# jolars/sgdnet

Hardware: AMD Instinct MI355X
Metric: saga_epochs_per_sec (higher is better)
Workload: dtype f64

## Files before the change

### include/sgdnet_hip.h

```cpp
#ifndef SGDNET_HIP_H_
#define SGDNET_HIP_H_

#include <stdint.h>

#ifdef __cplusplus
extern "C" {
#endif

#define SGDNET_ABI_VERSION 6

#define SGDNET_OK          0
#define SGDNET_EINVAL     -1
#define SGDNET_ENODEVICE  -2
#define SGDNET_EHIP       -3
#define SGDNET_ENOMEM     -4
#define SGDNET_EUNSUPPORTED -5
#define SGDNET_ESTREAM    -6

#define SGDNET_GAUSSIAN    0
#define SGDNET_BINOMIAL    1
#define SGDNET_MULTINOMIAL 2
#define SGDNET_MGAUSSIAN   3

#define SGDNET_RIDGE       0
// ... 119 lines not shown
int sgdnet_solver_set_penalty(sgdnet_solver* s, int penalty, double gamma, double alpha, double beta);

int sgdnet_solver_get_state(sgdnet_solver* s, int which, double* host);
int sgdnet_solver_set_state(sgdnet_solver* s, int which, const double* host);

int sgdnet_solver_generate_stream(sgdnet_solver* s, sgdnet_rng* rng, int64_t count);

int sgdnet_solver_get_stream(sgdnet_solver* s, uint32_t* host, int64_t offset, int64_t count);

int sgdnet_solver_upload_stream(sgdnet_solver* s, const uint32_t* host, int64_t count);

int sgdnet_solver_run(sgdnet_solver* s, int mode, int64_t batch,
                      int64_t stream_offset, int64_t draws_per_epoch,
                      unsigned max_epochs, double tol,
                      unsigned* epochs_run, int* converged, double* losses);

int sgdnet_solver_enqueue_epochs(sgdnet_solver* s, int64_t batch, int64_t stream_offset,
                                 int64_t draws_per_epoch, int n_epochs);
int sgdnet_solver_sync(sgdnet_solver* s);

int sgdnet_solver_rng_layout(sgdnet_solver* s, int64_t draws_per_run);
int sgdnet_solver_rng_open(sgdnet_solver* s, sgdnet_rng* rng, int64_t draws_per_epoch, int generators);
int sgdnet_solver_rng_next(sgdnet_solver* s, int64_t* stream_offset);
int sgdnet_solver_rng_done(sgdnet_solver* s);
int sgdnet_solver_rng_close(sgdnet_solver* s, sgdnet_rng* rng);

int sgdnet_solver_profile_epoch(sgdnet_solver* s, int64_t batch, int64_t stream_offset,
                                int64_t draws_per_epoch, double* gather_ms, int* gather_launches,
                                double* sweep_ms, int* sweep_launches);

int sgdnet_solver_epoch_timing(sgdnet_solver* s, int enable, double* sum_ms, int* launches);

int sgdnet_solver_gather_form(const sgdnet_solver* s, int64_t batch);

int sgdnet_solver_link_peers(sgdnet_solver** solvers, int n);
int sgdnet_solver_peer_info_bytes(void);
int sgdnet_solver_peer_info(sgdnet_solver* s, void* out);
int sgdnet_solver_link_ipc(sgdnet_solver* s, int rank, int n_ranks, const void* infos);
int sgdnet_solver_set_cu_budget(sgdnet_solver* s, int cus);

int sgdnet_solver_deviance(sgdnet_solver* s, double* out);

int sgdnet_solver_snapshot(sgdnet_solver* s);
int sgdnet_solver_export_delta(sgdnet_solver* s, void* device_buf);
int sgdnet_solver_apply_merged(sgdnet_solver* s, const void* device_buf, double w_weight);
int64_t sgdnet_solver_delta_len(const sgdnet_solver* s);

void* sgdnet_solver_stream(sgdnet_solver* s);
int sgdnet_solver_export_delta_async(sgdnet_solver* s, void* device_buf);
int sgdnet_solver_export_delta_weighted_async(sgdnet_solver* s, void* device_buf, double weight);
int sgdnet_solver_apply_merged_async(sgdnet_solver* s, const void* device_buf, double w_weight);

int64_t sgdnet_solver_sync_buffer_len(const sgdnet_solver* s);
int sgdnet_solver_sync_bind(sgdnet_solver* s, void* device_buf);
int sgdnet_solver_sync_begin(sgdnet_solver* s, int64_t stream_offset, int64_t draws_local_per_epoch);
int sgdnet_solver_sync_gather(sgdnet_solver* s, int64_t t0_local, int64_t m_local, int round);
int sgdnet_solver_sync_sweep(sgdnet_solver* s, int64_t m_global, int64_t m_local, int round);
int sgdnet_solver_sync_end(sgdnet_solver* s, int rounds);

int sgdnet_solver_set_virtual_shards(sgdnet_solver* s, int n_shards);
int sgdnet_solver_set_merge_period(sgdnet_solver* s, int64_t draws_per_shard);

int sgdnet_solver_set_n_total(sgdnet_solver* s, int64_t n_total);

int sgdnet_solver_convergence(sgdnet_solver* s, double tol, int* converged);

// ... 132 lines not shown
```

### sgdnet_amd/_lib.py

```python
import ctypes as C
import os
import sys

_HERE = os.path.dirname(os.path.abspath(__file__))
LIB_PATH = os.environ.get("SGDNET_LIB_PATH") or os.path.join(_HERE, "lib", "libsgdnet_hip.so")

EXPORTS = [
    "sgdnet_abi_version", "sgdnet_last_error", "sgdnet_device_count", "sgdnet_set_option", "sgdnet_get_option",
    "sgdnet_fit_sparse", "sgdnet_fit_dense",
    "sgdnet_rng_seed", "sgdnet_rng_unif", "sgdnet_rng_fill", "sgdnet_rng_jump_poly", "sgdnet_rng_jump",
    "sgdnet_solver_create", "sgdnet_solver_destroy", "sgdnet_solver_set_penalty",
    "sgdnet_solver_get_state", "sgdnet_solver_set_state", "sgdnet_solver_upload_stream",
    "sgdnet_solver_generate_stream", "sgdnet_solver_get_stream",
    "sgdnet_solver_run", "sgdnet_solver_enqueue_epochs", "sgdnet_solver_sync",
    "sgdnet_solver_profile_epoch", "sgdnet_solver_deviance", "sgdnet_solver_snapshot",
    "sgdnet_solver_export_delta", "sgdnet_solver_apply_merged", "sgdnet_solver_delta_len",
    "sgdnet_solver_convergence", "sgdnet_solver_last_change", "sgdnet_auto_batch", "sgdnet_shard_window",
    "sgdnet_solver_gather_form", "sgdnet_solver_stream", "sgdnet_solver_export_delta_async",
    "sgdnet_solver_apply_merged_async", "sgdnet_solver_sync_buffer_len", "sgdnet_solver_sync_bind",
    "sgdnet_solver_sync_begin", "sgdnet_solver_sync_gather", "sgdnet_solver_sync_sweep",
    "sgdnet_solver_sync_end", "sgdnet_solver_set_n_total",
    "sgdnet_solver_export_delta_weighted_async", "sgdnet_solver_set_virtual_shards", "sgdnet_solver_set_merge_period",
    "sgdnet_score_sparse", "sgdnet_score_dense", "sgdnet_predict_sparse", "sgdnet_predict_dense",
    "sgdnet_auc_sparse", "sgdnet_auc_dense", "sgdnet_auc_sparse_rng", "sgdnet_auc_dense_rng",
    "sgdnet_solver_link_peers", "sgdnet_solver_set_cu_budget", "sgdnet_solver_epoch_timing",
    "sgdnet_solver_peer_info_bytes", "sgdnet_solver_peer_info", "sgdnet_solver_link_ipc",
    "sgdnet_solver_rng_layout", "sgdnet_solver_rng_open", "sgdnet_solver_rng_next", "sgdnet_solver_rng_done", "sgdnet_solver_rng_close",
    "sgdnet_gradient_sparse", "sgdnet_gradient_dense", "sgdnet_covariance_max_features",
    "sgdnet_setup_probe_sparse", "sgdnet_setup_probe_dense",
    "sgdnet_cv_covariance_dense", "sgdnet_cv_covariance_sparse", "sgdnet_newton_max_features",
    "sgdnet_newton_probe_dense", "sgdnet_newton_probe_sparse",
    "sgdnet_cv_newton_dense", "sgdnet_cv_newton_sparse", "sgdnet_mcovariance_max_features",
    "sgdnet_mnewton_max_features",
]
ABI_VERSION = 6
MEASURES = {"deviance": 0, "mse": 1, "mae": 2, "class": 3, "auc": 4}

FAMILIES = {"gaussian": 0, "binomial": 1, "multinomial": 2, "mgaussian": 3}
PENALTIES = {"ridge": 0, "elasticnet": 1, "grouplasso": 2}
MODES = {"exact": 0, "batched": 1, "auto": 2, "covariance": 3}
MODE_NEWTON = 4
MODE_MCOVARIANCE = 5
MODE_MNEWTON = 6

UNIF_FN = C.CFUNCTYPE(C.c_double, C.c_void_p)
LOSSES_FN = C.CFUNCTYPE(None, C.c_void_p, C.c_int, C.POINTER(C.c_double), C.c_int)


class Csc(C.Structure):
    _fields_ = [("n_rows", C.c_int64), ("n_cols", C.c_int64),
                ("colptr", C.POINTER(C.c_int32)), ("rowidx", C.POINTER(C.c_int32)),
                ("values", C.POINTER(C.c_double))]


class Rng(C.Structure):
    _fields_ = [("mti", C.c_uint32), ("mt", C.c_uint32 * 624)]


class Control(C.Structure):
    _fields_ = [("debug", C.c_int), ("elasticnet_mix", C.c_double), ("family", C.c_int),
                ("intercept", C.c_int), ("is_sparse", C.c_int),
                ("lambda_", C.POINTER(C.c_double)), ("n_lambda_user", C.c_int),
                ("lambda_min_ratio", C.c_double), ("max_iter", C.c_uint), ("n_lambda", C.c_int),
                ("n_classes", C.c_int), ("standardize", C.c_int),
                ("standardize_response", C.c_int), ("tol", C.c_double),
                ("type_multinomial", C.c_int),
# ... 103 lines not shown
    L.sgdnet_solver_enqueue_epochs.argtypes = [C.c_void_p, C.c_int64, C.c_int64, C.c_int64, C.c_int]
    L.sgdnet_solver_sync.argtypes = [C.c_void_p]
    L.sgdnet_solver_profile_epoch.argtypes = [C.c_void_p, C.c_int64, C.c_int64, C.c_int64,
                                              C.POINTER(C.c_double), C.POINTER(C.c_int),
                                              C.POINTER(C.c_double), C.POINTER(C.c_int)]
    L.sgdnet_solver_deviance.argtypes = [C.c_void_p, C.POINTER(C.c_double)]
    L.sgdnet_solver_snapshot.argtypes = [C.c_void_p]
    L.sgdnet_solver_export_delta.argtypes = [C.c_void_p, C.c_void_p]
    L.sgdnet_solver_apply_merged.argtypes = [C.c_void_p, C.c_void_p, C.c_double]
    L.sgdnet_solver_delta_len.argtypes = [C.c_void_p]
    L.sgdnet_solver_stream.argtypes = [C.c_void_p]
    L.sgdnet_solver_stream.restype = C.c_void_p
    L.sgdnet_solver_export_delta_async.argtypes = [C.c_void_p, C.c_void_p]
    L.sgdnet_solver_apply_merged_async.argtypes = [C.c_void_p, C.c_void_p, C.c_double]
    L.sgdnet_solver_sync_buffer_len.argtypes = [C.c_void_p]
    L.sgdnet_solver_sync_buffer_len.restype = C.c_int64
    L.sgdnet_solver_sync_bind.argtypes = [C.c_void_p, C.c_void_p]
    L.sgdnet_solver_sync_begin.argtypes = [C.c_void_p, C.c_int64, C.c_int64]
    L.sgdnet_solver_sync_gather.argtypes = [C.c_void_p, C.c_int64, C.c_int64, C.c_int]
    L.sgdnet_solver_sync_sweep.argtypes = [C.c_void_p, C.c_int64, C.c_int64, C.c_int]
    L.sgdnet_solver_sync_end.argtypes = [C.c_void_p, C.c_int]
    L.sgdnet_solver_set_n_total.argtypes = [C.c_void_p, C.c_int64]
    L.sgdnet_solver_set_virtual_shards.argtypes = [C.c_void_p, C.c_int]
    L.sgdnet_solver_set_merge_period.argtypes = [C.c_void_p, C.c_int64]
    L.sgdnet_solver_link_peers.argtypes = [C.POINTER(C.c_void_p), C.c_int]
    L.sgdnet_solver_set_cu_budget.argtypes = [C.c_void_p, C.c_int]
    L.sgdnet_solver_peer_info.argtypes = [C.c_void_p, C.c_void_p]
    L.sgdnet_solver_link_ipc.argtypes = [C.c_void_p, C.c_int, C.c_int, C.c_void_p]
    L.sgdnet_solver_epoch_timing.argtypes = [C.c_void_p, C.c_int, C.POINTER(C.c_double), C.POINTER(C.c_int)]
    L.sgdnet_solver_export_delta_weighted_async.argtypes = [C.c_void_p, C.c_void_p, C.c_double]
    L.sgdnet_solver_convergence.argtypes = [C.c_void_p, C.c_double, C.POINTER(C.c_int)]
    L.sgdnet_solver_last_change.argtypes = [C.c_void_p, C.POINTER(C.c_double), C.POINTER(C.c_double)]
    L.sgdnet_solver_gather_form.argtypes = [C.c_void_p, C.c_int64]
    L.sgdnet_auto_batch.argtypes = [C.c_double, C.c_double]
    L.sgdnet_auto_batch.restype = C.c_int64
    L.sgdnet_shard_window.argtypes = [C.c_int64, C.c_int64]
    L.sgdnet_shard_window.restype = C.c_int64
    L.sgdnet_fit_sparse.argtypes = [C.POINTER(Csc), C.POINTER(C.c_double), C.c_int,
                                    C.POINTER(Control), C.POINTER(Result)]
    L.sgdnet_fit_dense.argtypes = [C.POINTER(C.c_double), C.c_int64, C.c_int64,
                                   C.POINTER(C.c_double), C.c_int, C.POINTER(Control),
                                   C.POINTER(Result)]
    L.sgdnet_rng_fill.argtypes = [C.POINTER(Rng), C.c_uint32, C.POINTER(C.c_uint32), C.c_int64]
    L.sgdnet_solver_rng_open.argtypes = [C.c_void_p, C.POINTER(Rng), C.c_int64, C.c_int]
    L.sgdnet_solver_rng_layout.argtypes = [C.c_void_p, C.c_int64]
    L.sgdnet_solver_rng_next.argtypes = [C.c_void_p, C.POINTER(C.c_int64)]
    L.sgdnet_solver_rng_done.argtypes = [C.c_void_p]
    L.sgdnet_solver_rng_close.argtypes = [C.c_void_p, C.POINTER(Rng)]
    L.sgdnet_rng_jump_poly.argtypes = [C.c_uint64, C.POINTER(C.c_uint32)]
    L.sgdnet_rng_jump.argtypes = [C.POINTER(Rng), C.POINTER(C.c_uint32), C.POINTER(Rng)]
    L.sgdnet_rng_jump.restype = None
    _grad_tail = [C.POINTER(C.c_double), C.c_int, C.c_int, C.c_int, C.POINTER(C.c_double), C.POINTER(C.c_double),
                  C.c_int, C.c_int, C.POINTER(C.c_double), C.POINTER(C.c_double)]
    L.sgdnet_gradient_sparse.argtypes = [C.POINTER(Csc)] + _grad_tail
    L.sgdnet_gradient_dense.argtypes = [C.POINTER(C.c_double), C.c_int64, C.c_int64] + _grad_tail
    L.sgdnet_setup_probe_sparse.argtypes = [C.POINTER(Csc), C.c_int, C.POINTER(C.c_double), C.c_int, C.POINTER(C.c_double),
                                            C.c_int, C.c_int, C.c_int, C.POINTER(SetupProbe)]
    L.sgdnet_setup_probe_dense.argtypes = [C.POINTER(C.c_double), C.c_int64, C.c_int64, C.c_int, C.POINTER(C.c_double), C.c_int,
                                           C.c_int64, C.c_int64, C.c_int, C.POINTER(SetupProbe)]
    L.sgdnet_newton_probe_dense.argtypes = [C.POINTER(C.c_double), C.c_int64, C.c_int64, C.c_int, C.POINTER(NewtonProbe)]
    L.sgdnet_newton_probe_sparse.argtypes = [C.POINTER(Csc), C.c_int, C.POINTER(NewtonProbe)]
    _cv_tail = [C.POINTER(C.c_double), C.POINTER(C.c_int32), C.c_int, C.c_int, C.POINTER(Control), C.c_int, C.POINTER(C.c_double),
                C.POINTER(C.c_double), C.POINTER(CvCovResult)]
    L.sgdnet_cv_covariance_dense.argtypes = [C.POINTER(C.c_double), C.c_int64, C.c_int64] + _cv_tail
    L.sgdnet_cv_covariance_sparse.argtypes = [C.POINTER(Csc)] + _cv_tail
    _cv_tail = _cv_tail[:-1] + [C.POINTER(CvNewtonResult)]
# ... 16 lines not shown
```

### sgdnet_amd/csrc/batched_geometry.hpp

```cpp
#pragma once

#include <hip/hip_ext.h>

#include <type_traits>

#include "common.hpp"

#ifndef SGDNET_BIN_BLOCK
#define SGDNET_BIN_BLOCK 1024
#endif
#ifndef SGDNET_BIN_W
#define SGDNET_BIN_W 8
#endif
#ifndef SGDNET_RANGE_BLOCK
#define SGDNET_RANGE_BLOCK 512
#endif
#ifndef SGDNET_LDS_BLOCK
#define SGDNET_LDS_BLOCK 1024
#endif

namespace sgdnet {

constexpr int kGroup = 16;
constexpr int kBlock = 256;

constexpr int kD0Slots = 256;

constexpr int kCStride = 128;
constexpr uint32_t kIdMask = 0x1fffffffu;
constexpr int kInReg8 = 16;

constexpr int kLdsBlock = SGDNET_LDS_BLOCK;
constexpr int kDenseBlock = 256;
constexpr int kDenseVsBlock = 1024;
constexpr int kTileF = 64;

constexpr int kSlabElems = 32;
constexpr int kSlabGroups = kBlock / kSlabElems;

constexpr int kSyncLine = 32;
constexpr int kSyncGo = 0, kSyncExit = 1, kSyncStart = 2, kSyncCnt1 = 3, kSyncCnt2 = kSyncCnt1 + 8,
              kSyncXcd = kSyncCnt2 + 8;
constexpr int kFusedMaxBps = 128;
constexpr int kSyncLines = kSyncXcd + 8;
constexpr int kSyncSticky = kSyncLines;
constexpr int kSyncSeq = kSyncLines + 1;
constexpr int kFusedChunks = 3;
constexpr long long kFusedStartTicks = 2000000;
constexpr long long kFusedWaitTicks = 200000000;

struct __attribute__((aligned(16))) BinEntry {
  uint32_t t;
  uint32_t j;
  double x;
};
static_assert(sizeof(BinEntry) == 16, "bin entries are 16 bytes");

constexpr int kBinBlock = SGDNET_BIN_BLOCK;
constexpr int kBinDraws = kBinBlock / 2;
constexpr int kBinEntCap = 7 * kBinBlock;
constexpr int kBinW = SGDNET_BIN_W;
constexpr int kRangeBlock = SGDNET_RANGE_BLOCK;
constexpr size_t kRangeLdsBytes = 64 * 1024;

constexpr size_t kLdsPerCu = 160 * 1024;
constexpr size_t kLdsStaticReserve = 2 * 1024;
constexpr size_t kLdsTableMax = 80 * 1024;
constexpr int kLdsCap = 96 * 1024;
constexpr int kLdsAll = (int)(kLdsPerCu - kLdsStaticReserve);

template <typename F>
static int with_class_width(int kw, F&& f) {
  if (kw == 1) return f(std::integral_constant<int, 1>{});
  if (kw == 4) return f(std::integral_constant<int, 4>{});
  return f(std::integral_constant<int, 16>{});
}

static inline unsigned clamped_grid(int64_t work, int64_t per_block, int64_t most) {
  const int64_t grid = (work + per_block - 1) / per_block;
// ... 32 lines not shown
```

### sgdnet_amd/csrc/batched_plan.cpp

```cpp
#include <mutex>
#include <set>
#include <utility>

#include "batched_geometry.hpp"
#include "r_rng_bodies.hpp"

namespace sgdnet {

int batched_max_classes() { return 64; }

int lds_target_grid(const SagaDev& d) {
  static const int forced = exp_env_int("SGDNET_LDS_GRID", 0);
  if (forced > 0) return forced;
  const int cus = d.cu_budget > 0 && d.cu_budget < 256 ? d.cu_budget : 256;
  const int g = cus - d.cu_reserve;
  return g < 64 ? 64 : g;
}

size_t binned_max_range_features(int K) { return kRangeLdsBytes / (sizeof(double) * (size_t)K); }

static size_t table_bytes(const SagaDev& d) { return sizeof(double) * (size_t)d.K * (size_t)d.p; }

int allow_dynamic_lds(const void* kernel, int bytes) {
  int dev = 0;
// ... 16 lines not shown

bool compact_eligible(const SagaDev& d) {
  static const int allow = exp_env_int("SGDNET_COMPACT", 1);
  if (!allow || d.K != 1 || d.Ky != 1 || d.xd || !d.ptr || d.p > 65536) return false;
  if (2 * sizeof(double) * (size_t)d.p + 16 + kLdsStaticReserve > (size_t)kLdsPerCu) return false;
  return (double)d.n * 2.0 * kCStride <= 48e9 && d.n < (int64_t)kIdMask;
}

int compact_entries(const SagaDev& d) { return d.family == SGDNET_BINOMIAL && d.y_binary ? 12 : 11; }

bool wants_binned(const SagaDev& d, int64_t batch) {
  static const int allow = exp_env_int("SGDNET_BINNED", 1);
  return allow && !d.xd && d.rec && d.idx && d.K <= 64 && !d.force_global && d.p < (1ll << 31) &&
         (d.K > 16 || (table_bytes(d) > kLdsTableMax && batch >= 4096));
}

bool wants_tiles(const SagaDev& d) { return d.xd && d.K <= 64 && (d.K > 16 || table_bytes(d) > kLdsTableMax); }

bool vs_eligible(const SagaDev& d) {
  if (d.V < 2 || d.K < 1 || d.K > 16 || (d.standardize && !(d.vcw && d.c)) || d.force_global || !d.vw) return false;
  const size_t table = table_bytes(d);
  if (d.xd) return table <= kLdsTableMax;
  if (d.K > 1) return d.rec && table <= kLdsTableMax;
  return 2 * table + 16 + kLdsStaticReserve <= kLdsPerCu;
}

static int vs_grid(const SagaDev& d) { return d.v_bps * d.V; }

static int64_t fused_slice(const SagaDev& d) { return 2 * ((d.p + 2 * (int64_t)d.v_bps - 1) / (2 * (int64_t)d.v_bps)); }
static size_t fused_lds_bytes(const SagaDev& d) {
  const int64_t part = (int64_t)(kLdsBlock / 64) * fused_slice(d);
  return sizeof(double) * (size_t)(d.p + (part > d.p ? part : d.p)) + 16;
}
size_t vs_fused_sync_words() { return (size_t)(kSyncLines + 2) * kSyncLine; }
size_t vs_fused_sync_sticky_word() { return (size_t)kSyncSticky * kSyncLine; }
size_t vs_fused_col_words() { return (size_t)kFusedMaxBps * kSyncLine; }
size_t vs_fused_exchange_doubles(const SagaDev& d, int n_shards) {
  return (size_t)n_shards * (size_t)(2 * d.p + 2) + (size_t)n_shards * kFusedMaxBps;
}
size_t vs_fused_publish_doubles(const SagaDev& d, int n_shards) { return (size_t)2 * n_shards * (size_t)(2 * d.p + 2); }

bool vs_fused_eligible(const SagaDev& d) {
  if (!vs_eligible(d) || d.K != 1 || d.xd || !d.cP || !lanes8_ok(d) || (d.p & 1) || !d.vsync || !d.vx || !d.vcol || !d.vpub) return false;
  if (d.v_bps < 1 || d.v_bps > kFusedMaxBps || d.V * d.v_bps > 1024) return false;
  if (fused_slice(d) > 2 * 64 * kFusedChunks) return false;
  if ((int64_t)d.V * d.v_bps * d.p * 8 >= (1ll << 31)) return false;
  return fused_lds_bytes(d) + kLdsStaticReserve <= kLdsPerCu;
}

static int vs_fused_rng_workgroups(const SagaDev& d) { return d.rngdev ? d.cu_reserve : 0; }

BatchPlan plan_batch(const SagaDev& d, int m, const PlanInputs& in) {
  BatchPlan g{};
  g.kw = class_width(d.K);
  const size_t table = table_bytes(d);
  if (d.V > 1 && vs_eligible(d)) {
    const int rng_wgs = vs_fused_rng_workgroups(d);
    g.slab_doubles = (int64_t)vs_grid(d) * d.K * d.p;
    if (in.fused && vs_fused_eligible(d) && vs_grid(d) + rng_wgs <= in.cus) {
      g.form = BatchForm::kFusedEpoch;
      g.grid = vs_grid(d) + rng_wgs;
      g.lds_bytes = fused_lds_bytes(d);
      if (rng_wgs > 0 && g.lds_bytes < kJumpLds) g.lds_bytes = kJumpLds;
      return g;
    }
    g.form = BatchForm::kShards;
    g.grid = vs_grid(d);
    int dpb = (m + d.v_bps - 1) / d.v_bps;
// ... 88 lines not shown
```

### sgdnet_amd/csrc/batched_shards.hip

```cpp
#include "batched_k1.hpp"
#include "r_rng_bodies.hpp"

namespace sgdnet {

template <int KMAX>
__global__ __launch_bounds__(kBlock) void saga_vs_sweep_kernel(SagaDev d, LamParams* lamp, int tail, int nfb) {
  __shared__ double part[kSlabGroups][kSlabElems];
  __shared__ double red[kBlock / 64];
  __shared__ double sh_d0[KMAX];
  const SweepParams q = load_sweep_params(d, lamp, tail, SweepOverride{0.0, 0.0, 0.0});
  const int K = KMAX == 1 ? 1 : d.K;
  const int F = kSlabElems / K;
  const int E = F * K;
  const int v = (int)blockIdx.x / nfb, fb = (int)blockIdx.x - v * nfb;
  const int64_t KP = (int64_t)K * d.p;
  const double n_d = d.v_size[v];
  const int e = threadIdx.x % kSlabElems, g = threadIdx.x / kSlabElems;
  const int64_t elem = (int64_t)fb * E + e;
  const int64_t j_own = (int64_t)fb * F + threadIdx.x;
  const bool updates = (int)threadIdx.x < F && j_own < d.p;
  double w_old[KMAX], g_old[KMAX], c_own = 0.0;
#pragma unroll
  for (int k = 0; k < KMAX; ++k) {
    w_old[k] = g_old[k] = 0.0;
// ... 172 lines not shown
}
__device__ __forceinline__ unsigned sync_load(unsigned* sync, int word) {
  return __hip_atomic_load(sync + word * kSyncLine, __ATOMIC_RELAXED, __HIP_MEMORY_SCOPE_AGENT);
}

__device__ __forceinline__ void fused_arrive(unsigned* sync, int word) {
  asm volatile("s_waitcnt vmcnt(0)" ::: "memory");
  __syncthreads();
  if (threadIdx.x == 0)
    __hip_atomic_fetch_add(sync + word * kSyncLine, 1u, __ATOMIC_RELAXED, __HIP_MEMORY_SCOPE_AGENT);
}

__device__ __forceinline__ bool fused_poll(unsigned* ctr, int word, unsigned target, LamParams* lamp, bool system = false,
                                           unsigned* sync = nullptr) {
  if (!sync) sync = ctr;
  const long long t0 = wall_clock64();
  for (unsigned spins = 1;; ++spins) {
    const unsigned now = system ? __hip_atomic_load(ctr + word * kSyncLine, __ATOMIC_RELAXED, __HIP_MEMORY_SCOPE_SYSTEM)
                                : sync_load(ctr, word);
    if (now >= target) return true;
    __builtin_amdgcn_s_sleep(4);
    if ((spins & 63u) == 0) {
      if (sync_load(sync, kSyncGo) != 1u) return false;
      if (wall_clock64() - t0 > kFusedWaitTicks) {
        __hip_atomic_store(sync + kSyncGo * kSyncLine, 3u, __ATOMIC_RELAXED, __HIP_MEMORY_SCOPE_AGENT);
        __hip_atomic_store(&lamp->fused_abort, 2, __ATOMIC_RELAXED, __HIP_MEMORY_SCOPE_AGENT);
        __hip_atomic_store(sync + kSyncSticky * kSyncLine, 2u, __ATOMIC_RELAXED, __HIP_MEMORY_SCOPE_AGENT);
        return false;
      }
    }
  }
}

__device__ __forceinline__ bool fused_start(unsigned* sync, LamParams* lamp, unsigned grid) {
  unsigned* go = sync + kSyncGo * kSyncLine;
  const long long t0 = wall_clock64();
  if (blockIdx.x == 0) {
    unsigned expect = 0u;
    for (;;) {
      if (sync_load(sync, kSyncStart) >= grid) {
        __hip_atomic_compare_exchange_strong(go, &expect, 1u, __ATOMIC_RELAXED, __ATOMIC_RELAXED, __HIP_MEMORY_SCOPE_AGENT);
        break;
      }
      if (sync_load(sync, kSyncGo) != 0u) break;
      if (wall_clock64() - t0 > kFusedStartTicks) {
        __hip_atomic_compare_exchange_strong(go, &expect, 2u, __ATOMIC_RELAXED, __ATOMIC_RELAXED, __HIP_MEMORY_SCOPE_AGENT);
        break;
      }
      __builtin_amdgcn_s_sleep(4);
    }
  } else {
    for (;;) {
      if (sync_load(sync, kSyncGo) != 0u) break;
      if (wall_clock64() - t0 > 2 * kFusedStartTicks) {
        unsigned expect = 0u;
        __hip_atomic_compare_exchange_strong(go, &expect, 2u, __ATOMIC_RELAXED, __ATOMIC_RELAXED, __HIP_MEMORY_SCOPE_AGENT);
        break;
      }
      __builtin_amdgcn_s_sleep(4);
    }
  }
  const unsigned decision = sync_load(sync, kSyncGo);
  if (decision != 1u && decision != 3u) {
    __hip_atomic_store(&lamp->fused_abort, 1, __ATOMIC_RELAXED, __HIP_MEMORY_SCOPE_AGENT);
    __hip_atomic_fetch_max(sync + kSyncSticky * kSyncLine, 1u, __ATOMIC_RELAXED, __HIP_MEMORY_SCOPE_AGENT);
  }
  return decision == 1u;
}

__device__ __forceinline__ double fused_block_sum(double a, double* red) {
  a = wave_sum(a);
  if ((threadIdx.x & 63) == 0) red[threadIdx.x >> 6] = a;
  __syncthreads();
  double t = 0.0;
#pragma unroll
  for (int wv = 0; wv < kLdsBlock / 64; ++wv) t += red[wv];
  __syncthreads();
  return t;
}

__device__ __forceinline__ void fused_leave(const SagaDev& d, LamParams* lamp, int nb, bool epoch_done) {
  asm volatile("s_waitcnt vmcnt(0)" ::: "memory");
  __syncthreads();
  if (threadIdx.x == 0) {
    unsigned* sync = d.vsync;
    if (epoch_done && blockIdx.x == 0) {
      end_epoch(lamp, nb);
      if (d.n_peers > 1) __hip_atomic_fetch_add(sync + kSyncSeq * kSyncLine, 1u, __ATOMIC_RELAXED, __HIP_MEMORY_SCOPE_AGENT);
    }
    const unsigned prev = __hip_atomic_fetch_add(sync + kSyncExit * kSyncLine, 1u, __ATOMIC_RELAXED, __HIP_MEMORY_SCOPE_AGENT);
    if (prev + 1u == gridDim.x) {
      for (int wd = 0; wd < kSyncLines; ++wd)
        __hip_atomic_store(sync + wd * kSyncLine, 0u, __ATOMIC_RELAXED, __HIP_MEMORY_SCOPE_AGENT);
      if (!(d.n_peers > 1))
        for (int wd = 0; wd < kFusedMaxBps; ++wd)
          __hip_atomic_store(d.vcol + wd * kSyncLine, 0u, __ATOMIC_RELAXED, __HIP_MEMORY_SCOPE_AGENT);
      if (d.rngdev && lamp->rng_generate) d.rngdev->gen += 1u;
    }
  }
}

template <bool kPeers>
__global__ __launch_bounds__(kLdsBlock) void saga_vs_epoch_kernel(SagaDev d, LamParams* lamp, int nb, int every) {
  extern __shared__ __attribute__((aligned(16))) double Dl[];
  __shared__ int ticket_counter;
  __shared__ int sh_ok;
  __shared__ double sh_red[kLdsBlock / 64];
  __shared__ double sh_val[4];
  const int tid = threadIdx.x;
  const int64_t p = d.p;
  const int64_t P2 = p >> 1;
  const int S = d.v_bps, V = d.V;
  if ((int)blockIdx.x >= V * S) {
    if (d.rngdev && lamp->rng_generate) {
      const RngDev* R = d.rngdev;
      const unsigned gen = R->gen;
      uint32_t* lds = reinterpret_cast<uint32_t*>(Dl);
      const int rb = (int)blockIdx.x - V * S, nrb = (int)gridDim.x - V * S;
      mt_state_body(rb, nrb, reinterpret_cast<uint32_t(*)[2][kMtN + 1]>(lds), R->state[gen & 1u], R->ends,
                    R->stream + (int64_t)(gen & 1u) * R->n, R->n, R->seg, R->gens);
      __syncthreads();
      mt_jump_body(rb, nrb, lds, R->state[gen & 1u], R->state[(gen + 1u) & 1u], R->poly, R->gens);
    }
    fused_leave(d, lamp, nb, false);
    return;
  }
  const int v = (int)blockIdx.x % V, wi = (int)blockIdx.x / V;
  const int F = 2 * (int)((p + 2 * S - 1) / (2 * S));
  const int j0 = wi * F;
  const int jn = p - j0 < F ? (p - j0 > 0 ? (int)(p - j0) : 0) : F;
  double* Wl = Dl + p;
  f64x2_t* D2 = reinterpret_cast<f64x2_t*>(Dl);
  f64x2_t* W2 = reinterpret_cast<f64x2_t*>(Wl);
  const int penalty = lamp->penalty;
  __shared__ double sh_par[10];
  if (tid == 0) {
    sh_par[0] = lamp->gamma;
    sh_par[1] = lamp->beta;
    sh_par[2] = lamp->r_full;
// ... 19 lines not shown
  double* vGv = d.vG + (int64_t)v * p;
  double* refv = d.vx + (int64_t)v * L;
  double* cwp = d.vx + (int64_t)V * L;
  unsigned* sync = d.vsync;
  const __amdgpu_buffer_rsrc_t rs_slab = fused_rsrc(d.slab, (int64_t)V * S * p * 8);
  const __amdgpu_buffer_rsrc_t rs_w = fused_rsrc(vwv, p * 8);
  const uint32_t* const stream_v = d.stream + sbase + (int64_t)v * dps;
  typedef K1CompactT<true> K1Epoch;
  const double* const draw_par = sh_par + 6;

#ifdef SGDNET_PHASE_TIMING
  unsigned long long ph_t = 0;
  if (d.dbg && tid == 0) d.dbg[(size_t)blockIdx.x * 16 + 14] = ph_t = phase_stamp();
#define FPH(slot)                                                 \
  do {                                                            \
    if (d.dbg && tid == 0) {                                      \
      const unsigned long long now = phase_stamp();               \
      d.dbg[(size_t)blockIdx.x * 16 + (slot)] += now - ph_t;      \
      d.dbg[(size_t)blockIdx.x * 16 + 15] = ph_t = now;           \
    }                                                             \
  } while (0)
#else
#define FPH(slot) ((void)0)
#endif
  if (tid == 0) {
    const unsigned xcc = __builtin_amdgcn_s_getreg((3 << 11) | 20) & 15u;
    __hip_atomic_fetch_or(sync + (kSyncXcd + v) * kSyncLine, 1u << xcc, __ATOMIC_RELAXED, __HIP_MEMORY_SCOPE_AGENT);
    asm volatile("s_waitcnt vmcnt(0)" ::: "memory");
    __hip_atomic_fetch_add(sync + kSyncStart * kSyncLine, 1u, __ATOMIC_RELAXED, __HIP_MEMORY_SCOPE_AGENT);
    sh_ok = fused_start(sync, lamp, (unsigned)(V * S)) ? 1 : 0;
    if (sh_ok) {
      const unsigned mask = sync_load(sync, kSyncXcd + v);
      sh_ok = (mask & (mask - 1u)) == 0u ? 3 : 1;
    }
  }
  for (int64_t i = tid; i < P2; i += kLdsBlock) D2[i] = f64x2_t{0.0, 0.0};
  __syncthreads();
  bool done = false;
  bool alive = sh_ok != 0;
  unsigned col_base = 0u;
  if (kPeers) {
    int merges = 0;
    for (int r = 0; r < nb; ++r) merges += (r + 1 == nb || (r + 1) % every == 0) ? 1 : 0;
    col_base = sync_load(sync, kSyncSeq) * (unsigned)merges;
  }
  const bool local = (sh_ok & 2) != 0 && d.vs_xcd_local != 0;
  int mi = 0;
  uint32_t s_first = 0u, s_second = 0u;
  if (alive) {
    const int m0 = (int)(dps < m_full ? dps : m_full);
    K1Epoch nx;
    nx.begin(d, stream_v, m0, wi, S, &ticket_counter);
    s_first = nx.s_cur;
    s_second = nx.s_nxt;
  }
  for (int r = 0; alive && r < nb; ++r) {
    const int64_t t0 = (int64_t)r * m_full;
    const int m = (int)(dps - t0 < m_full ? dps - t0 : m_full);
    const bool tail = m != m_full;
    const bool last = r + 1 == nb;
    const bool merge_due = last || (r + 1) % every == 0;

    if (tid == 0) ticket_counter = K1Epoch::static_tickets();
    K1Epoch cg;
    cg.init(d, stream_v + t0, m, wi, S, &ticket_counter);
    cg.raw = raw_words;
    cg.par = draw_par;
    cg.s_cur = s_first;
    cg.s_nxt = s_second;
    cg.tag_first();
    int ts = threadIdx.x;
    asm volatile("" : "+v"(ts));
    double cw = 0.0, bv = 0.0;
    if ((ts >> 6) == 0) {
      if (std_x && r > 0)
        for (int k = ts & 63; k < S; k += 64) cw += ld_sc1(cwp + v * kFusedMaxBps + k);
      bv = r == 0 ? d.b[0] : ld_sc1(d.vb + v);
    }
    {
// ... 22 lines not shown
      double a = 0.0;
      for (int64_t j = ts; j < p; j += kLdsBlock) a += d.c[j] * Wl[j];
      a = fused_block_sum(a, sh_red);
      if (ts == 0) sh_val[0] -= a;
      __syncthreads();
    }
    const double b0 = sh_val[0];
    FPH(0);

    const double gct = cg.run(d, b0, Wl, Dl);
    __syncthreads();
    FPH(1);
    int tq = threadIdx.x;
    asm volatile("" : "+v"(tq));
    const int lane = tq & 63, wave = tq >> 6;
    const int64_t t0n = t0 + m_full;
    const int mn = (int)(dps - t0n < m_full ? dps - t0n : m_full);

    {
      const uint32_t base = (uint32_t)(((int64_t)blockIdx.x * p) * 8);
      for (int64_t i = tq; i < P2; i += kLdsBlock) {
        st2_shard(D2[i], rs_slab, base + (uint32_t)(i * 16), local);
        D2[i] = f64x2_t{0.0, 0.0};
      }
      const double t = wave_sum(gct);
      if (lane == 0) sh_red[wave] = t;
      __syncthreads();
      if (tq == 0) {
        double tot = 0.0;
        for (int wv = 0; wv < kLdsBlock / 64; ++wv) tot += sh_red[wv];
        st_shard(d.vd0 + blockIdx.x, tot, local);
      }
    }
    fused_arrive(sync, kSyncCnt1 + v);
    FPH(2);
    const bool upd = tq < jn;
    const bool icpt = wi == 0 && tq == jn;
    const bool act = upd || icpt;
    const int64_t j = j0 + tq;
    const int64_t oa = upd ? j : 2 * p, ob = upd ? p + j : 2 * p + 1;
    double* const rep_a = upd ? vGv + j : d.vgb + v;
    double* const rep_b = upd ? vwv + j : d.vb + v;
    const double* const own_a = upd ? d.G + j : d.gb;
    const double* const own_b = upd ? d.w + j : d.b;
    double a_old = 0.0, b_old = 0.0, c_own = 0.0, ra = 0.0, rb = 0.0;
    if (act) {
      a_old = r == 0 ? *own_a : ld_sc1(rep_a);
      b_old = r == 0 ? *own_b : ld_sc1(rep_b);
      if (std_x && upd) c_own = d.c[j];
      if (merge_due) {
        ra = mi == 0 ? *own_a : ld_sc1(refv + oa);
        rb = mi == 0 ? *own_b : ld_sc1(refv + ob);
      }
    }
    if (tq == 0) sh_ok = fused_poll(sync, kSyncCnt1 + v, (unsigned)S * (unsigned)(r + 1), lamp) ? 1 : 0;
    __syncthreads();
    if (!sh_ok) break;
    FPH(3);

    {
      double gsum = 0.0;
      if (wave == kLdsBlock / 64 - 1)
        for (int k = lane; k < S; k += 64) gsum += ld_sc1(d.vd0 + k * V + v);
      f64x2_t acc[kFusedChunks];
#pragma unroll
      for (int c = 0; c < kFusedChunks; ++c) acc[c] = f64x2_t{0.0, 0.0};
      for (int k = wave; k < S; k += 2 * (kLdsBlock / 64)) {
        const bool two = k + kLdsBlock / 64 < S;
        const uint32_t o0 = (uint32_t)((((int64_t)(k * V + v)) * p + j0) * 8);
        const uint32_t o1 = (uint32_t)((((int64_t)((k + kLdsBlock / 64) * V + v)) * p + j0) * 8);
        f64x2_t a0[kFusedChunks], a1[kFusedChunks];
#pragma unroll
        for (int c = 0; c < kFusedChunks; ++c) {
          const int pi = c * 64 + lane;
          a0[c] = a1[c] = f64x2_t{0.0, 0.0};
          if (2 * pi < jn) {
            a0[c] = ld2_sc1(rs_slab, o0 + (uint32_t)(pi * 16));
            if (two) a1[c] = ld2_sc1(rs_slab, o1 + (uint32_t)(pi * 16));
          }
        }
#pragma unroll
        for (int c = 0; c < kFusedChunks; ++c) {
          acc[c] += a0[c];
          acc[c] += a1[c];
        }
      }
#pragma unroll
      for (int c = 0; c < kFusedChunks; ++c) {
// ... 76 lines not shown
        for (int u = 0; u < 8; ++u) {
          if (u < V) {
            const double wt = (PR ? PR->vsize[q][u] : d.v_size[u]) / tot_all;
            ma += wt * (xa[u] - ra);
            mb += wt * (xb[u] - rb);
          }
        }
      }
      if (act) {
        a_new = ma;
        b_new = mb;
        st_sc1(refv + oa, ma);
        st_sc1(refv + ob, mb);
        if (last && v == 0) {
          *const_cast<double*>(own_a) = ma;
          *const_cast<double*>(own_b) = mb;
        }
      }
      ++mi;
      FPH(5);
    }
    if (act) {
      st_shard(rep_a, a_new, local);
      st_shard(rep_b, b_new, local);
    }
    if (std_x) {
      const double a = fused_block_sum(upd ? c_own * b_new : 0.0, sh_red);
      if (tq == 0) st_shard(cwp + v * kFusedMaxBps + wi, a, local);
    }
    if (last) {
      done = true;
      break;
    }
    fused_arrive(sync, kSyncCnt2 + v);
    FPH(6);
    {
      K1Epoch nx;
      nx.begin(d, stream_v + t0n, mn, wi, S, &ticket_counter);
      s_first = nx.s_cur;
      s_second = nx.s_nxt;
    }
    if (tq == 0) sh_ok = fused_poll(sync, kSyncCnt2 + v, (unsigned)S * (unsigned)(r + 1), lamp) ? 1 : 0;
    __syncthreads();
    if (!sh_ok) break;
    FPH(7);
  }

  fused_leave(d, lamp, nb, done);
}

int launch_vs_broadcast(const SagaDev& d, hipStream_t st) {
  const int64_t len = 2 * (int64_t)d.K * d.p + 2 * d.K;
  return launch_kernel(saga_vs_broadcast_kernel, dim3(clamped_grid(len, kBlock, 1024)), dim3(kBlock), 0, 0, st, nullptr,
                       nullptr, d);
}

int launch_vs_cw(const SagaDev& d, hipStream_t st) {
  if (!d.standardize) return SGDNET_OK;
  return launch_kernel(saga_vs_cw_kernel, dim3(d.V * d.K), dim3(kBlock), 0, 0, st, nullptr, nullptr, d);
}

int launch_vs_merge(const SagaDev& d, int final_merge, hipStream_t st, LamParams* epoch_end, int batches) {
  const int64_t len = 2 * (int64_t)d.K * d.p + 2 * d.K;
  return launch_kernel(saga_vs_merge_kernel, dim3(clamped_grid(len, kBlock, 1024)), dim3(kBlock), 0, 0, st, nullptr,
                       nullptr, d, final_merge, epoch_end, batches);
}

int launch_vs_sweep(const SagaDev& d, const BatchPlan& g, LamParams* lam, int tail, hipStream_t st, hipEvent_t ev0,
                    hipEvent_t ev1) {
  const int F = kSlabElems / d.K;
  const int nfb = (int)((d.p + F - 1) / F);
  return with_class_width(g.kw, [&](auto kw) {
    return launch_kernel(saga_vs_sweep_kernel<decltype(kw)::value>, dim3(nfb * d.V), dim3(kBlock), 0, 0, st, ev0, ev1, d,
                         lam, tail, nfb);
  });
// ... 12 lines not shown
```

### sgdnet_amd/csrc/common.hpp

```cpp
#pragma once

#include <hip/hip_runtime.h>
#include <stdint.h>

#include "sgdnet_hip.h"

#ifdef SGDNET_EXPERIMENTS
#define SGD_ABLATE(d, bits) (((d).ablate & (bits)) != 0)
#else
#define SGD_ABLATE(d, bits) false
#endif

#include <stdlib.h>

namespace sgdnet {

void set_error(const char* fmt, ...);

#ifdef SGDNET_EXPERIMENTS
inline int exp_env_int(const char* name, int dflt) {
  const char* e = getenv(name);
  return e ? atoi(e) : dflt;
}
inline const char* exp_env_str(const char* name) { return getenv(name); }
// ... 202 lines not shown
};
struct PlanInputs {
  int64_t batch;
  bool bins_disabled;
  bool fused;
  int cus;
};
BatchPlan plan_batch(const SagaDev& d, int m, const PlanInputs& in);
bool wants_binned(const SagaDev& d, int64_t batch);
bool wants_tiles(const SagaDev& d);
bool vs_eligible(const SagaDev& d);
bool vs_fused_eligible(const SagaDev& d);
int launch_batch_gather(const SagaDev& d, const BatchPlan& g, LamParams* lam, int64_t t0_in_epoch, int m,
                        int batch_id_offset, hipStream_t st, hipEvent_t ev0 = nullptr, hipEvent_t ev1 = nullptr);
int launch_batch_sweep(const SagaDev& d, const BatchPlan& g, LamParams* lam, int penalty, int tail, int batch_id_offset,
                       hipStream_t st, hipEvent_t ev0 = nullptr, hipEvent_t ev1 = nullptr, double ov_r = 0.0,
                       double ov_ls = 0.0, double ov_m = 0.0);
int launch_vs_gather(const SagaDev& d, const BatchPlan& g, LamParams* lam, int64_t t0_in_epoch, int m, hipStream_t st,
                     hipEvent_t ev0 = nullptr, hipEvent_t ev1 = nullptr, int batch_index = 0);
int launch_vs_sweep(const SagaDev& d, const BatchPlan& g, LamParams* lam, int tail, hipStream_t st,
                    hipEvent_t ev0 = nullptr, hipEvent_t ev1 = nullptr);
int launch_vs_epoch(const SagaDev& d, const BatchPlan& g, LamParams* lam, int nb, int every, hipStream_t st,
                    hipEvent_t ev0 = nullptr, hipEvent_t ev1 = nullptr);
int allow_dynamic_lds(const void* kernel, int bytes);
template <typename F>
int allow_dynamic_lds(F* kernel, int bytes) { return allow_dynamic_lds(reinterpret_cast<const void*>(kernel), bytes); }
int launch_cw_init(const SagaDev& d, const LamParams* lam, hipStream_t st);
int launch_epoch_end(LamParams* lam, int batches, hipStream_t st);
int launch_vs_broadcast(const SagaDev& d, hipStream_t st);
int launch_vs_merge(const SagaDev& d, int final_merge, hipStream_t st, LamParams* epoch_end = nullptr, int batches = 0);
int launch_vs_cw(const SagaDev& d, hipStream_t st);
size_t vs_fused_sync_words();
size_t vs_fused_sync_sticky_word();
size_t vs_fused_col_words();
size_t vs_fused_publish_doubles(const SagaDev& d, int n_shards);
size_t vs_fused_exchange_doubles(const SagaDev& d, int n_shards);
bool compact_eligible(const SagaDev& d);
int launch_pack_compact(const SagaDev& d, char* P, char* Q, uint32_t* meta, hipStream_t st);
int compact_entries(const SagaDev& d);
int launch_m_move(const SagaDev& d, int to_record, hipStream_t st);

int launch_convergence(const SagaDev& d, LamParams* lam, hipStream_t st);
int launch_loss(const SagaDev& d, LamParams* lam, bool sparse, hipStream_t st);
int launch_delta_export(const SagaDev& d, const double* ref, double* out, double weight, hipStream_t st);
int launch_delta_apply(const SagaDev& d, double* ref, const double* merged, double w_weight, hipStream_t st);
int batched_max_classes();
int lds_target_grid(const SagaDev& d);
int launch_col_count(const SagaDev& d, int64_t nnz, unsigned* counts, hipStream_t st);
int launch_wpad_refresh(const SagaDev& d, hipStream_t st);
int launch_range_moment(const SagaDev& d, const uint16_t* feat_range, unsigned long long* sumsq, int R, hipStream_t st);
size_t binned_max_range_features(int K);
int launch_rng_fill(const uint32_t* state_in, uint32_t* state_out, uint32_t n_samples, uint32_t* out,
                    int64_t count, hipStream_t st, int n_shards = 0, const double* shard_size = nullptr,
                    int gens = 1, int64_t run_len = 0, int convert = 1, int narrow_cus = 0, int wgs = 0);
int launch_rng_convert(uint32_t* out, int64_t count, uint32_t n_samples, hipStream_t st, int n_shards,
                       const double* shard_size, int64_t run_len, int narrow_cus = 0);

bool mt_jump_poly(uint64_t J, uint32_t* out624);
void mt_jump_host(const sgdnet_rng* in, const uint32_t* poly624, sgdnet_rng* out);
int launch_rng_unif(const uint32_t* state_in, uint32_t* state_out, uint32_t* raw, double* out, int64_t count, hipStream_t st);
int launch_rng_jump(const uint32_t* state_in, uint32_t* state_out, const uint32_t* poly_dev, int gens,
                    hipStream_t st, int max_wgs = 0);
int rng_generators_per_workgroup();

}
```

### sgdnet_amd/csrc/solver_epoch.cpp

```cpp
#include <math.h>
#include <stdlib.h>
#include <stdio.h>
#include <string.h>

#include <algorithm>
#include <chrono>
#include <vector>

#include "solver_state.hpp"

namespace sgdnet {

static bool lam_on_device(const sgdnet_solver* s) {
  if (!s->lam_dev_valid) return false;
  const LamParams &a = s->lam, &b = s->lam_dev_mirror;
  return a.penalty == b.penalty && a.gamma == b.gamma && a.alpha == b.alpha && a.beta == b.beta && a.r_full == b.r_full &&
         a.ls_full == b.ls_full && a.r_tail == b.r_tail && a.ls_tail == b.ls_tail && a.m_full == b.m_full &&
         a.m_tail == b.m_tail && a.stream_base == b.stream_base && a.stream_wrap == b.stream_wrap &&
         a.draws_per_epoch == b.draws_per_epoch && a.batch_seq == b.batch_seq && a.stream_raw == b.stream_raw &&
         a.rng_generate == b.rng_generate;
}

static void lam_advance(sgdnet_solver* s, int64_t draws, int batches) {
  for (LamParams* q : {&s->lam, &s->lam_dev_mirror}) {
// ... 599 lines not shown
  int ng = 0;
  for (size_t i = 0; i + 3 < ev.size(); i += 4) {
    float ms = 0.f;
    SGD_HIP_TRY(hipEventElapsedTime(&ms, ev[i], ev[i + 1]));
    g += ms;
    SGD_HIP_TRY(hipEventElapsedTime(&ms, ev[i + 2], ev[i + 3]));
    w += ms;
    ++ng;
  }
#ifdef SGDNET_PHASE_TIMING
  rc = phase_report_batched(s, batch, fused_prof);
  if (rc) return rc;
#endif
  if (gather_ms) *gather_ms = g;
  if (gather_launches) *gather_launches = ng;
  if (sweep_ms) *sweep_ms = w;
  if (sweep_launches) *sweep_launches = ng;
  return SGDNET_OK;
}

int sgdnet_solver_gather_form(const sgdnet_solver* s, int64_t batch) {
  if (!s || batch < 1) return 0;
  const BatchPlan g = plan(s, batch, batch);
  if (g.form == BatchForm::kFusedEpoch) return 3;
  if (g.form == BatchForm::kBinned) return 2;
  if (g.form == BatchForm::kShards) {
    SagaDev d = s->d;
    d.V = 0;
    return plan_batch(d, (int)batch, PlanInputs{batch, s->bin_disabled, false, s->cus}).slab_doubles > 0 ? 1 : 0;
  }
  return g.slab_doubles > 0 ? 1 : 0;
}

int sgdnet_solver_last_change(const sgdnet_solver* s, double* max_change, double* max_size) {
  if (!s || !max_change || !max_size) return SGDNET_EINVAL;
  *max_change = s->last_change;
  *max_size = s->last_size;
  return SGDNET_OK;
}

int sgdnet_solver_epoch_timing(sgdnet_solver* s, int enable, double* sum_ms, int* launches) {
  if (!s) return SGDNET_EINVAL;
  SGD_HIP_TRY(hipSetDevice(s->device));
  SGD_HIP_TRY(hipStreamSynchronize(s->st));
  double tot = 0.0;
  int cnt = 0;
  for (size_t i = 0; i + 1 < s->epoch_ev.size(); i += 2) {
    float ms = 0.f;
    if (hipEventElapsedTime(&ms, s->epoch_ev[i], s->epoch_ev[i + 1]) == hipSuccess) {
      tot += ms;
      ++cnt;
    }
  }
  for (hipEvent_t e : s->epoch_ev) (void)hipEventDestroy(e);
  s->epoch_ev.clear();
  s->time_epochs = enable != 0;
  if (sum_ms) *sum_ms = tot;
  if (launches) *launches = cnt;
  return SGDNET_OK;
}

int sgdnet_solver_convergence(sgdnet_solver* s, double tol, int* converged) {
  if (!s || !converged) return SGDNET_EINVAL;
  SGD_HIP_TRY(hipSetDevice(s->device));
  return device_convergence(s, tol, converged);
}
// ... 82 lines not shown
```

### sgdnet_amd/solver.py

```python
import ctypes as C

import numpy as np

from . import _lib
from ._lib import FAMILIES, MODES, PENALTIES, check, dptr

STATE = {"w": 0, "intercept": 1, "g_memory": 2, "g_sum": 3, "g_sum_intercept": 4}


class RRng:

    def __init__(self, seed, sample_kind="Rejection"):
        if sample_kind not in ("Rejection", "Rounding"):
            raise ValueError("sample_kind must be 'Rejection' or 'Rounding'")
        self.sample_kind = sample_kind
        self._L = _lib.load()
        self.state = _lib.Rng()
        self._L.sgdnet_rng_seed(C.byref(self.state), C.c_uint32(seed))

    def unif(self, count=1):
        return np.array([self._L.sgdnet_rng_unif(C.byref(self.state)) for _ in range(count)])

    def stream(self, n_samples, count):
        out = np.empty(count, dtype=np.uint32)
# ... 257 lines not shown
    def apply_merged(self, device_ptr, w_weight):
        check(self._L.sgdnet_solver_apply_merged(self._h, C.c_void_p(device_ptr), w_weight))

    def sync_buffer_len(self):
        return int(self._L.sgdnet_solver_sync_buffer_len(self._h))

    def sync_bind(self, device_ptr):
        check(self._L.sgdnet_solver_sync_bind(self._h, C.c_void_p(device_ptr) if device_ptr else None))

    def sync_begin(self, stream_offset, draws_local):
        check(self._L.sgdnet_solver_sync_begin(self._h, stream_offset, draws_local))

    def sync_gather(self, t0_local, m_local, rnd):
        check(self._L.sgdnet_solver_sync_gather(self._h, t0_local, m_local, rnd))

    def sync_sweep(self, m_global, m_local, rnd):
        check(self._L.sgdnet_solver_sync_sweep(self._h, m_global, m_local, rnd))

    def sync_end(self, rounds):
        check(self._L.sgdnet_solver_sync_end(self._h, rounds))

    def set_virtual_shards(self, n_shards):
        check(self._L.sgdnet_solver_set_virtual_shards(self._h, n_shards))
        self.n_shards = n_shards

    def set_merge_period(self, draws_per_shard):
        check(self._L.sgdnet_solver_set_merge_period(self._h, draws_per_shard))

    def epoch_timing(self, enable):
        ms, cnt = C.c_double(0), C.c_int(0)
        check(self._L.sgdnet_solver_epoch_timing(self._h, int(bool(enable)), C.byref(ms), C.byref(cnt)))
        return ms.value, cnt.value

    def peer_info(self):
        buf = C.create_string_buffer(self._L.sgdnet_solver_peer_info_bytes())
        check(self._L.sgdnet_solver_peer_info(self._h, buf))
        return buf.raw

    def link_ipc(self, rank, infos):
        blob = b"".join(infos)
        check(self._L.sgdnet_solver_link_ipc(self._h, int(rank), len(infos), C.c_char_p(blob)))

    def set_cu_budget(self, cus):
        check(self._L.sgdnet_solver_set_cu_budget(self._h, int(cus)))

    def sharded_stream(self, rngs, epochs):
        from .parallel import shard_bounds
        V = len(rngs)
        dps = self.n // V
        out = np.empty(epochs * V * dps, dtype=np.uint32)
        for e in range(epochs):
            for v in range(V):
                lo, hi = shard_bounds(self.n, V, v)
                seg = rngs[v].stream(hi - lo, dps).astype(np.int64) + lo
                out[(e * V + v) * dps:(e * V + v + 1) * dps] = seg
        return out

    def set_n_total(self, n_total):
        check(self._L.sgdnet_solver_set_n_total(self._h, n_total))

    def stream_handle(self):
        return int(self._L.sgdnet_solver_stream(self._h) or 0)

    def export_delta_async(self, device_ptr, weight=1.0):
        check(self._L.sgdnet_solver_export_delta_weighted_async(self._h, C.c_void_p(device_ptr), weight))

# ... 3 lines not shown
```

Baseline: 1324.

## Replace atomic counter barriers with per-block stamped flag lines in fused epoch

In the fused virtual-shard epoch kernel, when shards are XCD-local and there are no peers, each block now writes a monotonically increasing stamp into its own slot of a flag line instead of doing a fetch-add on a shared counter. Waiters poll all slots at once with a wavefront ballot. A per-launch stamp base is advanced at kernel exit, and a transport word plus a query API record which barrier path was used. This is meant to cut atomic contention and polling latency at the two per-round barriers, at the cost of extra sync lines and more complex abort and timeout handling.

```diff
diff --git a/include/sgdnet_hip.h b/include/sgdnet_hip.h
--- a/include/sgdnet_hip.h
+++ b/include/sgdnet_hip.h
@@ -175,6 +175,8 @@
 int sgdnet_solver_epoch_timing(sgdnet_solver* s, int enable, double* sum_ms, int* launches);
 
 int sgdnet_solver_gather_form(const sgdnet_solver* s, int64_t batch);
+
+int sgdnet_solver_fused_transport(sgdnet_solver* s, int* out);
 
 int sgdnet_solver_link_peers(sgdnet_solver** solvers, int n);
 int sgdnet_solver_peer_info_bytes(void);
diff --git a/sgdnet_amd/_lib.py b/sgdnet_amd/_lib.py
--- a/sgdnet_amd/_lib.py
+++ b/sgdnet_amd/_lib.py
@@ -31,7 +31,7 @@
     "sgdnet_cv_covariance_dense", "sgdnet_cv_covariance_sparse", "sgdnet_newton_max_features",
     "sgdnet_newton_probe_dense", "sgdnet_newton_probe_sparse",
     "sgdnet_cv_newton_dense", "sgdnet_cv_newton_sparse", "sgdnet_mcovariance_max_features",
-    "sgdnet_mnewton_max_features",
+    "sgdnet_mnewton_max_features", "sgdnet_solver_fused_transport",
 ]
 ABI_VERSION = 6
 MEASURES = {"deviance": 0, "mse": 1, "mae": 2, "class": 3, "auc": 4}
@@ -201,6 +201,7 @@
     L.sgdnet_solver_convergence.argtypes = [C.c_void_p, C.c_double, C.POINTER(C.c_int)]
     L.sgdnet_solver_last_change.argtypes = [C.c_void_p, C.POINTER(C.c_double), C.POINTER(C.c_double)]
     L.sgdnet_solver_gather_form.argtypes = [C.c_void_p, C.c_int64]
+    L.sgdnet_solver_fused_transport.argtypes = [C.c_void_p, C.POINTER(C.c_int)]
     L.sgdnet_auto_batch.argtypes = [C.c_double, C.c_double]
     L.sgdnet_auto_batch.restype = C.c_int64
     L.sgdnet_shard_window.argtypes = [C.c_int64, C.c_int64]
diff --git a/sgdnet_amd/csrc/batched_geometry.hpp b/sgdnet_amd/csrc/batched_geometry.hpp
--- a/sgdnet_amd/csrc/batched_geometry.hpp
+++ b/sgdnet_amd/csrc/batched_geometry.hpp
@@ -45,6 +45,10 @@
 constexpr int kSyncLines = kSyncXcd + 8;
 constexpr int kSyncSticky = kSyncLines;
 constexpr int kSyncSeq = kSyncLines + 1;
+constexpr int kSyncStamp = kSyncLines + 2;
+constexpr int kSyncTransport = kSyncLines + 3;
+constexpr int kSyncFlag1 = kSyncLines + 4, kSyncFlag2 = kSyncFlag1 + 8;
+constexpr int kSyncAllLines = kSyncFlag2 + 8;
 constexpr int kFusedChunks = 3;
 constexpr long long kFusedStartTicks = 2000000;
 constexpr long long kFusedWaitTicks = 200000000;
diff --git a/sgdnet_amd/csrc/batched_plan.cpp b/sgdnet_amd/csrc/batched_plan.cpp
--- a/sgdnet_amd/csrc/batched_plan.cpp
+++ b/sgdnet_amd/csrc/batched_plan.cpp
@@ -72,8 +72,9 @@
   const int64_t part = (int64_t)(kLdsBlock / 64) * fused_slice(d);
   return sizeof(double) * (size_t)(d.p + (part > d.p ? part : d.p)) + 16;
 }
-size_t vs_fused_sync_words() { return (size_t)(kSyncLines + 2) * kSyncLine; }
+size_t vs_fused_sync_words() { return (size_t)kSyncAllLines * kSyncLine; }
 size_t vs_fused_sync_sticky_word() { return (size_t)kSyncSticky * kSyncLine; }
+size_t vs_fused_sync_transport_word() { return (size_t)kSyncTransport * kSyncLine; }
 size_t vs_fused_col_words() { return (size_t)kFusedMaxBps * kSyncLine; }
 size_t vs_fused_exchange_doubles(const SagaDev& d, int n_shards) {
   return (size_t)n_shards * (size_t)(2 * d.p + 2) + (size_t)n_shards * kFusedMaxBps;
diff --git a/sgdnet_amd/csrc/batched_shards.hip b/sgdnet_amd/csrc/batched_shards.hip
--- a/sgdnet_amd/csrc/batched_shards.hip
+++ b/sgdnet_amd/csrc/batched_shards.hip
@@ -228,6 +228,33 @@
   }
 }
 
+__device__ __forceinline__ void flag_arrive(unsigned* line, int wi, unsigned stamp) {
+  asm volatile("s_waitcnt vmcnt(0)" ::: "memory");
+  __syncthreads();
+  if (threadIdx.x == 0) __hip_atomic_store(line + wi, stamp, __ATOMIC_RELAXED, __HIP_MEMORY_SCOPE_WAVEFRONT);
+}
+
+__device__ __forceinline__ bool flag_poll(unsigned* line, int lane, int S, unsigned stamp, unsigned* sync, LamParams* lamp) {
+  const long long t0 = wall_clock64();
+  for (unsigned spins = 1;; ++spins) {
+    unsigned now = stamp;
+    if (lane < S) now = __hip_atomic_load(line + lane, __ATOMIC_RELAXED, __HIP_MEMORY_SCOPE_AGENT);
+    if (__builtin_amdgcn_ballot_w64((int)(now - stamp) < 0) == 0ull) return true;
+    __builtin_amdgcn_s_sleep(4);
+    if ((spins & 63u) == 0) {
+      if (__builtin_amdgcn_readfirstlane(sync_load(sync, kSyncGo)) != 1u) return false;
+      if (wall_clock64() - t0 > kFusedWaitTicks) {
+        if (lane == 0) {
+          __hip_atomic_store(sync + kSyncGo * kSyncLine, 3u, __ATOMIC_RELAXED, __HIP_MEMORY_SCOPE_AGENT);
+          __hip_atomic_store(&lamp->fused_abort, 2, __ATOMIC_RELAXED, __HIP_MEMORY_SCOPE_AGENT);
+          __hip_atomic_store(sync + kSyncSticky * kSyncLine, 2u, __ATOMIC_RELAXED, __HIP_MEMORY_SCOPE_AGENT);
+        }
+        return false;
+      }
+    }
+  }
+}
+
 __device__ __forceinline__ bool fused_start(unsigned* sync, LamParams* lamp, unsigned grid) {
   unsigned* go = sync + kSyncGo * kSyncLine;
   const long long t0 = wall_clock64();
@@ -286,6 +313,9 @@
     }
     const unsigned prev = __hip_atomic_fetch_add(sync + kSyncExit * kSyncLine, 1u, __ATOMIC_RELAXED, __HIP_MEMORY_SCOPE_AGENT);
     if (prev + 1u == gridDim.x) {
+      const unsigned went = sync_load(sync, kSyncGo);
+      if (went == 1u || went == 3u)
+        __hip_atomic_fetch_add(sync + kSyncStamp * kSyncLine, (unsigned)nb, __ATOMIC_RELAXED, __HIP_MEMORY_SCOPE_AGENT);
       for (int wd = 0; wd < kSyncLines; ++wd)
         __hip_atomic_store(sync + wd * kSyncLine, 0u, __ATOMIC_RELAXED, __HIP_MEMORY_SCOPE_AGENT);
       if (!(d.n_peers > 1))
@@ -301,6 +331,7 @@
   extern __shared__ __attribute__((aligned(16))) double Dl[];
   __shared__ int ticket_counter;
   __shared__ int sh_ok;
+  __shared__ unsigned sh_stamp;
   __shared__ double sh_red[kLdsBlock / 64];
   __shared__ double sh_val[4];
   const int tid = threadIdx.x;
@@ -386,6 +417,7 @@
     if (sh_ok) {
       const unsigned mask = sync_load(sync, kSyncXcd + v);
       sh_ok = (mask & (mask - 1u)) == 0u ? 3 : 1;
+      sh_stamp = sync_load(sync, kSyncStamp);
     }
   }
   for (int64_t i = tid; i < P2; i += kLdsBlock) D2[i] = f64x2_t{0.0, 0.0};
@@ -399,6 +431,15 @@
     col_base = sync_load(sync, kSyncSeq) * (unsigned)merges;
   }
   const bool local = (sh_ok & 2) != 0 && d.vs_xcd_local != 0;
+  const bool flags = !kPeers && local && S <= kSyncLine;
+  if (alive && tid == 0) {
+    if (!kPeers && S <= kSyncLine) {
+      __hip_atomic_store(sync + (kSyncFlag1 + v) * kSyncLine + wi, sh_stamp, __ATOMIC_RELAXED, __HIP_MEMORY_SCOPE_WAVEFRONT);
+      __hip_atomic_store(sync + (kSyncFlag2 + v) * kSyncLine + wi, sh_stamp, __ATOMIC_RELAXED, __HIP_MEMORY_SCOPE_WAVEFRONT);
+    }
+    if (wi == 0)
+      __hip_atomic_store(sync + kSyncTransport * kSyncLine + v, flags ? 2u : 1u, __ATOMIC_RELAXED, __HIP_MEMORY_SCOPE_AGENT);
+  }
   int mi = 0;
   uint32_t s_first = 0u, s_second = 0u;
   if (alive) {
@@ -487,7 +528,10 @@
         st_shard(d.vd0 + blockIdx.x, tot, local);
       }
     }
-    fused_arrive(sync, kSyncCnt1 + v);
+    if (flags)
+      flag_arrive(sync + (kSyncFlag1 + v) * kSyncLine, wi, sh_stamp + (unsigned)(r + 1));
+    else
+      fused_arrive(sync, kSyncCnt1 + v);
     FPH(2);
     const bool upd = tq < jn;
     const bool icpt = wi == 0 && tq == jn;
@@ -508,7 +552,14 @@
         rb = mi == 0 ? *own_b : ld_sc1(refv + ob);
       }
     }
-    if (tq == 0) sh_ok = fused_poll(sync, kSyncCnt1 + v, (unsigned)S * (unsigned)(r + 1), lamp) ? 1 : 0;
+    if (flags) {
+      if (wave == 0) {
+        const bool ok = flag_poll(sync + (kSyncFlag1 + v) * kSyncLine, lane, S, sh_stamp + (unsigned)(r + 1), sync, lamp);
+        if (lane == 0) sh_ok = ok ? 1 : 0;
+      }
+    } else if (tq == 0) {
+      sh_ok = fused_poll(sync, kSyncCnt1 + v, (unsigned)S * (unsigned)(r + 1), lamp) ? 1 : 0;
+    }
     __syncthreads();
     if (!sh_ok) break;
     FPH(3);
@@ -651,7 +702,10 @@
       done = true;
       break;
     }
-    fused_arrive(sync, kSyncCnt2 + v);
+    if (flags)
+      flag_arrive(sync + (kSyncFlag2 + v) * kSyncLine, wi, sh_stamp + (unsigned)(r + 1));
+    else
+      fused_arrive(sync, kSyncCnt2 + v);
     FPH(6);
     {
       K1Epoch nx;
@@ -659,7 +713,14 @@
       s_first = nx.s_cur;
       s_second = nx.s_nxt;
     }
-    if (tq == 0) sh_ok = fused_poll(sync, kSyncCnt2 + v, (unsigned)S * (unsigned)(r + 1), lamp) ? 1 : 0;
+    if (flags) {
+      if (wave == 0) {
+        const bool ok = flag_poll(sync + (kSyncFlag2 + v) * kSyncLine, lane, S, sh_stamp + (unsigned)(r + 1), sync, lamp);
+        if (lane == 0) sh_ok = ok ? 1 : 0;
+      }
+    } else if (tq == 0) {
+      sh_ok = fused_poll(sync, kSyncCnt2 + v, (unsigned)S * (unsigned)(r + 1), lamp) ? 1 : 0;
+    }
     __syncthreads();
     if (!sh_ok) break;
     FPH(7);
diff --git a/sgdnet_amd/csrc/common.hpp b/sgdnet_amd/csrc/common.hpp
--- a/sgdnet_amd/csrc/common.hpp
+++ b/sgdnet_amd/csrc/common.hpp
@@ -258,6 +258,7 @@
 int launch_vs_cw(const SagaDev& d, hipStream_t st);
 size_t vs_fused_sync_words();
 size_t vs_fused_sync_sticky_word();
+size_t vs_fused_sync_transport_word();
 size_t vs_fused_col_words();
 size_t vs_fused_publish_doubles(const SagaDev& d, int n_shards);
 size_t vs_fused_exchange_doubles(const SagaDev& d, int n_shards);
diff --git a/sgdnet_amd/csrc/solver_epoch.cpp b/sgdnet_amd/csrc/solver_epoch.cpp
--- a/sgdnet_amd/csrc/solver_epoch.cpp
+++ b/sgdnet_amd/csrc/solver_epoch.cpp
@@ -655,6 +655,18 @@
   return g.slab_doubles > 0 ? 1 : 0;
 }
 
+int sgdnet_solver_fused_transport(sgdnet_solver* s, int* out) {
+  if (!s || !out) return SGDNET_EINVAL;
+  for (int v = 0; v < 8; ++v) out[v] = 0;
+  if (!s->d.vsync) return SGDNET_OK;
+  SGD_HIP_TRY(hipSetDevice(s->device));
+  unsigned words[8];
+  SGD_HIP_TRY(hipMemcpyAsync(words, s->d.vsync + vs_fused_sync_transport_word(), sizeof(words), hipMemcpyDeviceToHost, s->st));
+  SGD_HIP_TRY(hipStreamSynchronize(s->st));
+  for (int v = 0; v < 8; ++v) out[v] = (int)words[v];
+  return SGDNET_OK;
+}
+
 int sgdnet_solver_last_change(const sgdnet_solver* s, double* max_change, double* max_size) {
   if (!s || !max_change || !max_size) return SGDNET_EINVAL;
   *max_change = s->last_change;
diff --git a/sgdnet_amd/solver.py b/sgdnet_amd/solver.py
--- a/sgdnet_amd/solver.py
+++ b/sgdnet_amd/solver.py
@@ -313,6 +313,11 @@
         check(self._L.sgdnet_solver_epoch_timing(self._h, int(bool(enable)), C.byref(ms), C.byref(cnt)))
         return ms.value, cnt.value
 
+    def fused_transport(self):
+        out = (C.c_int * 8)()
+        check(self._L.sgdnet_solver_fused_transport(self._h, out))
+        return list(out)[:self.n_shards]
+
     def peer_info(self):
         buf = C.create_string_buffer(self._L.sgdnet_solver_peer_info_bytes())
         check(self._L.sgdnet_solver_peer_info(self._h, buf))
```

Result: slower. 1274 (-3.8%).
